# sanje2v/DualSuperResLearningForSemSeg

Measured on AMD Instinct MI355X. Metric: stage-3 train images/sec at 256x512->512x1024, higher is better.
Workload: dtype f32; 1 GPU; DSRL stage 3 (ResNet-101 OS16 + ASPP + SSSR/SISR decoders + FA loss), full train step, random-init weights, 256x512 input -> 512x1024 logits; global_batch=8, per_gpu_batch=8, parallelism=dp1, optimizer=SGD m0.9 wd5e-4 lr0.006

## Files before the change

dualsuperreslearningforsemseg_amd/csrc/conv_igemm.hip:

```cpp
#include "common.h"
#include "conv_common.h"
#include <algorithm>
#include <atomic>
#include <stdlib.h>
#include <string.h>
#include <mutex>
#include <vector>

namespace dsrl {

static std::atomic<int> g_conv_precision{-1};
constexpr int BK = 32;
constexpr int LDS_LD = 36;

template <int MR, int NR, int WGM, int WGN, bool DGRAD, int MINW = 2, bool = false>
__global__ __launch_bounds__(256, MINW) void conv_igemm_f32_kernel(const ConvArgs a) {
    constexpr int BM = 32 * MR * WGM, BN = 32 * NR * WGN;
    constexpr int A_IT = BM / 32, B_IT = BN / 32;
    extern __shared__ __attribute__((aligned(16))) float smem[];

    const int tid = threadIdx.x;
    const int lane = tid & 63;
    const int wave = __builtin_amdgcn_readfirstlane(tid >> 6);
    const int wm = wave / WGN, wn = wave % WGN;
// ... 1468 lines not shown
struct DgradBn { const float* x; const float* y; const float* mean; const float* invstd; float* stats; int ldx, ldy, relu; float gscale = 1.f; };
static bool bn_y_ok(const float* y, int ldy, int relu, int N, int H, int W, int C) {
    if (relu == 2) return y != nullptr && C % 32 == 0 && (long long)ldy >= (long long)N * H * W && ((uintptr_t)y % 4) == 0;
    return relu == 0 || (relu == 1 && y != nullptr && ldy >= C);
}
static int dgrad_impl(const float* dy, int lddy, const float* w, const float* wt_in, float* dx, int lddx,
                      int N, int H, int W, int C, int K, int R, int S, int stride, int pad, int dil,
                      void* ws, size_t ws_bytes, dsrl_stream_t stream, int accumulate, const DgradBn* bn = nullptr,
                      const unsigned* dy_amax = nullptr, const unsigned* w_amax = nullptr, const void* wt_split = nullptr,
                      const void* dy_planes = nullptr, const void* wt_planes = nullptr) {
    if (int e = check_conv(dy, w, dx, N, H, W, C, K, R, S, stride, pad, dil)) return e;
    const int Kp = pad4(K);
    DSRL_REQUIRE(lddy % 4 == 0 && ((uintptr_t)dy % 16) == 0, DSRL_E_UNSUPPORTED,
                 "conv2d_dgrad: lddy (%d) must be a multiple of 4 and dy 16-byte aligned", lddy);
    DSRL_REQUIRE(lddy >= Kp && lddx >= C, DSRL_E_BADARG, "conv2d_dgrad: ld smaller than (padded) channel count");
    hipStream_t st = (hipStream_t)stream;
    if (int e = bind_stream_device(st)) return e;
    const int Ho = out_size(H, R, stride, pad, dil), Wo = out_size(W, S, stride, pad, dil);
    const FwdPlan p = plan_dgrad(N, Ho, Wo, Kp, C, R, S, H, W, conv_planes(PASS_DGRAD), stride);
    const size_t wtb = dgrad_wt_bytes(C, K, R, S);
    DSRL_REQUIRE(ws && ws_bytes >= wtb + p.ws, DSRL_E_WORKSPACE, "conv2d_dgrad: workspace %zu < %zu", ws_bytes, wtb + p.ws);
    const float* wt = wt_in;
    float* slabs = (float*)((char*)ws + wtb);
    const bool use_planes = conv_f16() && dy_planes != nullptr && wt_planes != nullptr && dy_amax != nullptr && w_amax != nullptr && stride == 1 && K % 8 == 0 &&
                            planes_usable(K, lddy, dy_planes, wt_planes) && planes_cfg_supported((int)p.cfg, p.kg) && !(p.coop && p.splits > 1);
    const bool use_split = conv_f16() && wt_split != nullptr && w_amax != nullptr;
    if (wt == nullptr && use_planes) wt = (const float*)wt_planes;
    if (wt == nullptr && use_split) wt = (const float*)wt_split;
    if (wt == nullptr) {
        hipLaunchKernelGGL(weight_transpose_kernel, dim3((unsigned)ceil_div(C, 32), (unsigned)ceil_div(Kp, 32), (unsigned)(R * S)), dim3(256), 0, st,
                           w, (float*)ws, K, Kp, R * S, C);
        if (int e = launch_status("weight_transpose_kernel")) return e;
        wt = (const float*)ws;
    }
    ConvArgs a{};
    a.x = dy; a.w = wt; a.ldx = lddy; a.N = N; a.H = Ho; a.W = Wo; a.C = Kp; a.K = C; a.R = R; a.S = S; a.Ho = H; a.Wo = W;
    a.stride = stride; a.pad = pad; a.dil = dil; a.M = p.M; a.cchunks = p.cchunks; a.splits = p.splits; a.kg = p.kg; a.slab = (long long)p.M * C;
    {
        const long long xb = span_bytes((long long)N * Ho * Wo, lddy, Kp), wb = (long long)C * R * S * Kp * 4, yb = p.splits > 1 ? (long long)p.M * C * 4 : span_bytes(p.M, lddx, C);
        DSRL_REQUIRE_31(xb, "conv2d_dgrad(dy)"); DSRL_REQUIRE_31(wb, "conv2d_dgrad(w)"); DSRL_REQUIRE_31(yb, "conv2d_dgrad(dx)");
        a.x_bytes = (unsigned)xb; a.w_bytes = (unsigned)wb; a.y_bytes = (unsigned)yb;
    }
    if (conv_f16()) {
        OperandAmax am{dy_amax, w_amax};
        if (int e = resolve_amax(am, dy, lddy, (long long)N * Ho * Wo, Kp, w, C, (long long)K * R * S, C, ws, ws_bytes, wtb + p.ws, st, "conv2d_dgrad")) return e;
        a.amax_a = am.a; a.amax_b = am.b;
        if (wt_split != nullptr && w_amax != nullptr) {
            DSRL_REQUIRE(((uintptr_t)wt_split % 16) == 0, DSRL_E_BADARG, "conv2d_dgrad: unaligned pre-split filter");
            a.w = (const float*)wt_split; a.w_split = 1;
        }
        if (use_planes) {
            const long long pe = (long long)N * Ho * Wo * lddy, we = (long long)C * R * S * K;
            a.planes = conv_planes(PASS_DGRAD); a.w_split = 0;
            a.x = (const float*)dy_planes; a.w = (const float*)wt_planes;
            a.x_bytes = (unsigned)(span_bytes((long long)N * Ho * Wo, lddy, K) / 2); a.w_bytes = (unsigned)(we * 2);
            a.a_lo = (unsigned)planes_lo_offset(pe); a.b_lo = (unsigned)planes_lo_offset(we);
        }
    }
    ProfScope prof(prof_family(PASS_DGRAD), 2.0 * (double)dsrl_conv2d_inbounds_macs(N, H, W, C, K, R, S, stride, pad, dil), 4.0 * ((double)N * H * W * C + (double)K * R * S * C + (double)N * out_size(H, R, stride, pad, dil) * out_size(W, S, stride, pad, dil) * K), st);
    prof.shape("dgrad", N, H, W, C, K, R, stride, pad, dil);
    if (p.splits > 1 && !(p.coop && a.amax_a != nullptr && !a.planes && stride == 1)) {
        DSRL_REQUIRE(bn == nullptr, DSRL_E_UNSUPPORTED, "conv2d_dgrad: BatchNorm sums asked from a split-K launch that reduces through slabs");
        a.y = slabs; a.ldy = C; a.bias = nullptr;
        if (int e = launch_igemm<true>(a, p.cfg, st)) return e;
        const long long total = (long long)p.M * C;
        hipLaunchKernelGGL(splitk_reduce_kernel, dim3((unsigned)std::min<long long>(ceil_div(total, 256), 4096)), dim3(256), 0, st,
                           (const float*)slabs, p.splits, a.slab, p.M, C, (const float*)nullptr, dx, lddx, accumulate);
        return launch_status("splitk_reduce_kernel");
    }
    if (p.splits > 1) {
        a.coop_slab = slabs; a.tickets = const_cast<unsigned*>(a.amax_a);
        a.y_bytes = (unsigned)span_bytes(p.M, lddx, C);
    }
    a.y = dx; a.ldy = lddx; a.bias = nullptr; a.accumulate = accumulate;
    if (stride > 1 && conv_planes(PASS_DGRAD) && H % stride == 0 && W % stride == 0 && (W / stride) % 32 == 0 && knob("DSRL_DGRAD_PARITY", 1)) {
        int bm, bn_; cfg_dims(p.cfg, bm, bn_);
        const long long Mc = (long long)N * (H / stride) * (W / stride);
        if (Mc % bm == 0) { a.par = stride; a.Hh = H / stride; a.Wh = W / stride; a.pbm = bm; }
    }
    if (bn) {
        a.bn_x = bn->x; a.bn_y = bn->y; a.bn_mean = bn->mean; a.bn_invstd = bn->invstd; a.bstats = bn->stats; a.bn_ldx = bn->ldx; a.bn_ldy = bn->ldy; a.bn_relu = bn->relu;
        a.bn_gscale = bn->gscale;
        const bool y4 = bn->relu != 1 || (bn->ldy % 4 == 0 && ((uintptr_t)bn->y % 16) == 0);
        a.bn_fast = a.par == 0 && C % 4 == 0 && bn->ldx % 4 == 0 && y4 && ((uintptr_t)bn->x % 16) == 0 &&
                    ((uintptr_t)bn->mean % 16) == 0 && ((uintptr_t)bn->invstd % 16) == 0 && ((uintptr_t)bn->stats % 16) == 0;
    }
    return launch_igemm<true>(a, p.cfg, st);
}

extern "C" int dsrl_conv2d_dgrad(const float* dy, int lddy, const float* w, const float* wt_in, float* dx, int lddx,
                                 int N, int H, int W, int C, int K, int R, int S, int stride, int pad, int dil,
                                 void* ws, size_t ws_bytes, dsrl_stream_t stream) {
    return dgrad_impl(dy, lddy, w, wt_in, dx, lddx, N, H, W, C, K, R, S, stride, pad, dil, ws, ws_bytes, stream, 0);
}
extern "C" int dsrl_conv2d_dgrad_stats_parts(int N, int H, int W, int C, int K, int R, int S, int stride, int pad, int dil) {
    const int Ho = out_size(H, R, stride, pad, dil), Wo = out_size(W, S, stride, pad, dil);
    if (Ho <= 0 || Wo <= 0) return 0;
    const int npl = conv_planes(PASS_DGRAD);
    return fwd_stats_parts(plan_dgrad(N, Ho, Wo, pad4(K), C, R, S, H, W, npl, stride), npl, true);
}
extern "C" int dsrl_conv2d_dgrad_bnstats(const float* dy, int lddy, const float* w, const float* wt_in, float* dx, int lddx,
                                         int N, int H, int W, int C, int K, int R, int S, int stride, int pad, int dil,
                                         void* ws, size_t ws_bytes, const float* bn_x, int bn_ldx, const float* bn_y, int bn_ldy,
                                         const float* bn_mean, const float* bn_invstd, int bn_relu, float* bstats, int stats_parts, int accumulate,
                                         dsrl_stream_t stream) {
    DSRL_REQUIRE(bn_x && bn_mean && bn_invstd && bstats && bn_ldx >= C && bn_y_ok(bn_y, bn_ldy, bn_relu, N, H, W, C), DSRL_E_BADARG, "conv2d_dgrad_bnstats: bad BatchNorm arguments");
    DSRL_REQUIRE(dsrl_conv2d_dgrad_stats_parts(N, H, W, C, K, R, S, stride, pad, dil) == stats_parts && stats_parts > 0, DSRL_E_BADARG,
                 "conv2d_dgrad_bnstats: this launch writes %d row blocks of partials, the caller expects %d",
                 dsrl_conv2d_dgrad_stats_parts(N, H, W, C, K, R, S, stride, pad, dil), stats_parts);
    DgradBn bn{bn_x, bn_y, bn_mean, bn_invstd, bstats, bn_ldx, bn_ldy, bn_relu};
    return dgrad_impl(dy, lddy, w, wt_in, dx, lddx, N, H, W, C, K, R, S, stride, pad, dil, ws, ws_bytes, stream, accumulate ? 1 : 0, &bn);
}
extern "C" int dsrl_conv2d_dgrad_accumulate(const float* dy, int lddy, const float* w, const float* wt_in, float* dx, int lddx,
                                            int N, int H, int W, int C, int K, int R, int S, int stride, int pad, int dil,
                                            void* ws, size_t ws_bytes, dsrl_stream_t stream) {
    return dgrad_impl(dy, lddy, w, wt_in, dx, lddx, N, H, W, C, K, R, S, stride, pad, dil, ws, ws_bytes, stream, 1);
}

static void launch_wgrad(const WgradArgs& a_in, TileCfg cfg, int bm, int bn, dim3 grid, hipStream_t st) {
    const int npl = conv_planes(PASS_WGRAD);
    const bool f16 = conv_f16();
    if (npl) {
        WgradArgs a = a_in;
        make_magic(a.Ho * a.Wo, a.mHW, a.sHW);
        make_magic(a.Wo, a.mW, a.sW);
        const size_t stages = (size_t)2 * npl * 16 * ((bm * 2 + 64) + (bn * 2 + 64));
        const int kg = a.kg > 1 ? a.kg : 1;
        if (kg > 1) {
            const size_t lds = std::max(stages * kg, (size_t)kg * (bm / 32) * (bn / 32) / 4 * 16384 + 8192);
#define DSRL_LAUNCH_WKG(a_, b_, c_, d_, NPL_, KG_, F16_)                                                                            \
            {                                                                                                                        \
                static const hipError_t attr = hipFuncSetAttribute((const void*)conv_wgrad_split_kernel<a_, b_, c_, d_, NPL_, KG_, F16_>,  \
                                                                   hipFuncAttributeMaxDynamicSharedMemorySize, 144 * 1024);          \
                (void)attr;                                                                                                          \
                hipLaunchKernelGGL((conv_wgrad_split_kernel<a_, b_, c_, d_, NPL_, KG_, F16_>), grid, dim3(256 * KG_), lds, st, a);   \
            }
#define DSRL_WKG_BY_NPL(a_, b_, c_, d_, KG_) { if (f16 && npl == 1) DSRL_LAUNCH_WKG(a_, b_, c_, d_, 1, KG_, true) else if (f16) DSRL_LAUNCH_WKG(a_, b_, c_, d_, 2, KG_, true) else if (npl == 2) DSRL_LAUNCH_WKG(a_, b_, c_, d_, 2, KG_, false) else DSRL_LAUNCH_WKG(a_, b_, c_, d_, 3, KG_, false) }
            if (cfg == T64x64) DSRL_WKG_BY_NPL(1, 1, 2, 2, 2)
            else if (cfg == T128x64) DSRL_WKG_BY_NPL(2, 1, 2, 2, 2)
            else if (cfg == T64x128) DSRL_WKG_BY_NPL(1, 2, 2, 2, 2)
            else DSRL_WKG_BY_NPL(2, 2, 2, 2, 2)
#undef DSRL_WKG_BY_NPL
#undef DSRL_LAUNCH_WKG
            return;
        }
        const size_t lds = stages;
#define DSRL_LAUNCH_WGRAD(a_, b_, c_, d_)                                                                           \
        if (f16 && npl == 1) hipLaunchKernelGGL((conv_wgrad_split_kernel<a_, b_, c_, d_, 1, 1, true>), grid, dim3(256), lds, st, a); \
        else if (f16) hipLaunchKernelGGL((conv_wgrad_split_kernel<a_, b_, c_, d_, 2, 1, true>), grid, dim3(256), lds, st, a); \
        else if (npl == 2) hipLaunchKernelGGL((conv_wgrad_split_kernel<a_, b_, c_, d_, 2>), grid, dim3(256), lds, st, a); \
        else hipLaunchKernelGGL((conv_wgrad_split_kernel<a_, b_, c_, d_, 3>), grid, dim3(256), lds, st, a);
        DSRL_CFG_SWITCH(cfg, DSRL_LAUNCH_WGRAD)
#undef DSRL_LAUNCH_WGRAD
        return;
    }
    const size_t lds = (size_t)32 * (bm + bn) * sizeof(float);
#define DSRL_LAUNCH_WGRAD(a_, b_, c_, d_) hipLaunchKernelGGL((conv_wgrad_f32_kernel<a_, b_, c_, d_>), grid, dim3(256), lds, st, a_in)
    DSRL_CFG_SWITCH(cfg, DSRL_LAUNCH_WGRAD)
#undef DSRL_LAUNCH_WGRAD
}

namespace dsrl {
struct WgPlan { int Ho, Wo; long long P; TileCfg cfg; int bm, bn, ktiles, ctiles, psplits; TapList tl; size_t ws; bool w3; };
static int w3_psplits(long long tiles, long long chunks) {
    const int forced = knob("DSRL_FORCE_PSPLITS", 0);
    if (forced > 0) return (int)std::max<long long>(1, std::min<long long>(forced, chunks));
    long long sp = std::max<long long>(1, 2 * kNumCU / std::max<long long>(tiles, 1));
// ... 518 lines not shown
```

dualsuperreslearningforsemseg_amd/csrc/conv_split_kernel.h:

```cpp
#pragma once
#include "common.h"
#include "conv_common.h"

namespace dsrl {

template <int MR, int NR, int WGM, int WGN, bool DGRAD, int NPL, int KG = 1, int ARITH = 0, bool STR1 = false, bool COOP = false>
__global__ __launch_bounds__(64 * WGM * WGN * KG, KG == 1 ? 2 : 1)
void conv_igemm_split_kernel(const ConvArgs a) {
    const int stride = STR1 ? 1 : a.stride, par = STR1 ? 0 : a.par;
    constexpr bool F16 = ARITH != 0, PREB = ARITH == 2;
    constexpr int NT = 64 * WGM * WGN, RP = NT / 4;
    static_assert(NT == 256 || (NT == 512 && KG == 1), "4 waves per K group, or one group of 8 waves");
    static_assert(!F16 || NPL <= 2, "f16x3 carries two fp16 terms per operand, f16x1 one");
    using PT = Plane<F16>;
    using pl4 = typename PT::v4; using pl8 = typename PT::v8;
    const unsigned am_a = F16 ? amax_fetch(a.amax_a) : 0u, am_b = F16 ? amax_fetch(a.amax_b) : 0u;
    int sh_a = 0, sh_b = 0;
    constexpr int BM = 32 * MR * WGM, BN = 32 * NR * WGN;
    constexpr int A_IT = (BM + RP - 1) / RP, B_IT = (BN + RP - 1) / RP;
    constexpr int NV = A_IT + B_IT;
    constexpr bool FS = F16;
    constexpr int ROWB = FS ? 64 : 32;
    constexpr int STAGE = (BM + BN) * NPL * ROWB;
    extern __shared__ __attribute__((aligned(16))) float smem[];
    const int grp = KG > 1 ? __builtin_amdgcn_readfirstlane((int)(threadIdx.x >> 8)) : 0;
    char* const S0 = reinterpret_cast<char*>(smem) + grp * 2 * STAGE;
    char* const S1 = S0 + STAGE;

    const int tid = threadIdx.x & (NT - 1);
    const int lane = tid & 63;
    const int wave = __builtin_amdgcn_readfirstlane(tid >> 6);
    const int wm = wave / WGN, wn = wave % WGN;
    const int tile = a.xcd_remap ? xcd_contiguous(blockIdx.x, a.mtiles * a.ntiles) : blockIdx.x;
    const int tile_m = fast_div(tile, a.mNT, a.sNT);
    const int m0 = tile_m * BM, n0 = (tile - tile_m * a.ntiles) * BN, z = blockIdx.z;
    const int HoWo = a.Ho * a.Wo;

    const int c4 = tid & 3, r0 = tid >> 2;
    const bool b_rows = (BN % RP == 0) || r0 < BN;
    int a_n[A_IT], a_h[A_IT], a_w[A_IT];
    bool a_ok[A_IT];
#pragma unroll
    for (int i = 0; i < A_IT; ++i) {
        const int m = m0 + r0 + RP * i;
        a_ok[i] = m < a.M && (BM % RP == 0 || r0 + RP * i < BM);
        const int mm = a_ok[i] ? ((DGRAD && par) ? dgrad_pix(a, m) : m) : 0;
        const int n = fast_div(mm, a.mHW, a.sHW), rem = mm - n * HoWo;
        const int ho = fast_div(rem, a.mW, a.sW), wo = rem - ho * a.Wo;
        a_n[i] = n;
        if (DGRAD) { a_h[i] = ho + a.pad; a_w[i] = wo + a.pad; }
        else { a_h[i] = ho * stride - a.pad; a_w[i] = wo * stride - a.pad; }
    }
    const int RS = a.R * a.S;
    const __amdgpu_buffer_rsrc_t xr = __builtin_amdgcn_make_buffer_rsrc((void*)a.x, 0, (int)a.x_bytes, 0x00020000);
    const __amdgpu_buffer_rsrc_t wr = __builtin_amdgcn_make_buffer_rsrc((void*)a.w, 0, (int)a.w_bytes, 0x00020000);
    unsigned b_off[B_IT];
#pragma unroll
    for (int i = 0; i < B_IT; ++i) {
        const int k = n0 + r0 + RP * i;
        b_off[i] = (k < a.K && b_rows) ? (unsigned)k * (unsigned)(RS * a.C) * 4u : kOOB;
    }

    unsigned long long tapmask = 0ull;
    if (a.R * a.S == 1 && a.pad == 0) {
        tapmask = 1ull;
    } else {
        const int mf = m0, ml = min(m0 + BM, a.M) - 1;
        const int nf = fast_div(mf, a.mHW, a.sHW), nl = fast_div(ml, a.mHW, a.sHW);
        int hf = 0, hl = a.Ho - 1, wf = 0, wl = a.Wo - 1;
        if (nf == nl) {
            hf = fast_div(mf - nf * HoWo, a.mW, a.sW); hl = fast_div(ml - nl * HoWo, a.mW, a.sW);
            if (hf == hl) { wf = (mf - nf * HoWo) - hf * a.Wo; wl = (ml - nl * HoWo) - hl * a.Wo; }
        }
        const int pcls = (DGRAD && par) ? (m0 / BM) % (par * par) : 0;
        const int ph = (DGRAD && par) ? pcls / par : 0, pw = (DGRAD && par) ? pcls - ph * par : 0;
        if (DGRAD && par) { hf = 0; hl = a.Ho - 1; wf = 0; wl = a.Wo - 1; }
        for (int r = 0; r < a.R; ++r)
            for (int s = 0; s < a.S; ++s) {
                bool act;
                if (DGRAD) {
                    act = (hl + a.pad - r * a.dil >= 0) && (hf + a.pad - r * a.dil <= (a.H - 1) * stride) &&
                          (wl + a.pad - s * a.dil >= 0) && (wf + a.pad - s * a.dil <= (a.W - 1) * stride);
                    if (par) act = act && ((ph + a.pad - r * a.dil) % par == 0) && ((pw + a.pad - s * a.dil) % par == 0);
                } else {
                    act = (hl * stride - a.pad + r * a.dil >= 0) && (hf * stride - a.pad + r * a.dil <= a.H - 1) &&
                          (wl * stride - a.pad + s * a.dil >= 0) && (wf * stride - a.pad + s * a.dil <= a.W - 1);
                }
                if (act) tapmask |= 1ull << (r * a.S + s);
            }
    }
    const int ntaps = __builtin_popcountll(tapmask);
    const int nq = ntaps * a.cchunks;
    int q0 = 0, q1 = nq;
    if (a.splits > 1) { q0 = (int)((long long)nq * z / a.splits); q1 = (int)((long long)nq * (z + 1) / a.splits); }

    f32x16 acc[MR][NR];
#pragma unroll
    for (int i = 0; i < MR; ++i)
#pragma unroll
        for (int j = 0; j < NR; ++j)
#pragma unroll
            for (int e = 0; e < 16; ++e) acc[i][j][e] = 0.f;

    int cc = 0, tap = 0, pos = q0;
    unsigned long long rem_mask = tapmask;
    if (q0 < q1) {
        if (q0 > 0) {
            int skip = q0 / a.cchunks;
            cc = q0 - skip * a.cchunks;
            while (skip--) rem_mask &= rem_mask - 1;
        }
        tap = __builtin_ctzll(rem_mask);
    }
    auto advance = [&](int n) {
        cc += n; pos += n;
        while (cc >= a.cchunks) { cc -= a.cchunks; rem_mask &= rem_mask - 1; tap = __builtin_ctzll(rem_mask); }
    };
    unsigned a_off[A_IT];
    const unsigned inv_s = 65536u / (unsigned)a.S + 1u;
    auto set_tap = [&](int t) {
        const int r = a.S <= 8 ? (int)(((unsigned)t * inv_s) >> 16) : t / a.S, s = t - r * a.S;
#pragma unroll
        for (int i = 0; i < A_IT; ++i) {
            int hi, wi; bool ok = a_ok[i];
            if (DGRAD) {
                const int hn = a_h[i] - r * a.dil, wn_ = a_w[i] - s * a.dil;
                hi = hn / stride; wi = wn_ / stride;
                ok = ok && hn >= 0 && wn_ >= 0 && hi * stride == hn && wi * stride == wn_ && hi < a.H && wi < a.W;
            } else {
                hi = a_h[i] + r * a.dil; wi = a_w[i] + s * a.dil;
                ok = ok && hi >= 0 && hi < a.H && wi >= 0 && wi < a.W;
            }
            a_off[i] = ok ? (unsigned)((a_n[i] * a.H + hi) * a.W + wi) * (unsigned)a.ldx * 4u : kOOB;
        }
    };
    float4 R0[NV][2], R1[NV][2];
#pragma unroll
    for (int v = 0; v < NV; ++v) { R0[v][0] = R0[v][1] = R1[v][0] = R1[v][1] = make_float4(0.f, 0.f, 0.f, 0.f); }
    auto gload = [&](float4 (*R)[2], int t, int ch, unsigned dead) {
#pragma unroll
        for (int hf = 0; hf < 2; ++hf) {
            const int c = ch * 32 + hf * 16 + c4 * 4;
            const unsigned coff = (c < a.C ? (unsigned)c * 4u : kOOB) | dead;
            const unsigned woff = __builtin_elementwise_add_sat(coff, (unsigned)(t * a.C) * 4u);
#pragma unroll
            for (int i = 0; i < A_IT; ++i) R[i][hf] = buf_load4(xr, __builtin_elementwise_add_sat(a_off[i], coff));
#pragma unroll
            for (int i = 0; i < B_IT; ++i) R[A_IT + i][hf] = buf_load4(wr, __builtin_elementwise_add_sat(b_off[i], woff));
        }
    };
    int nextq = q0 + grp, tap_set = -1;
    auto issue = [&](float4 (*R)[2]) {
        const bool live = nextq < q1;
        if (live) {
            advance(nextq - pos);
            if (tap != tap_set) { set_tap(tap); tap_set = tap; }
            nextq += KG;
        }
        gload(R, tap, cc, live ? 0u : kOOB);
    };

    const int frag_row = lane & 31;
    auto wswz = [&](int hf) -> int { return FS ? (((((hf << 1) | (c4 >> 1)) ^ ((r0 >> 2) & 3)) << 4) + ((c4 & 1) << 3)) : ((((c4 >> 1) ^ ((r0 >> 3) & 1)) << 4) + ((c4 & 1) << 3)); };
    auto rswz = [&](int hf) -> int { return FS ? ((((hf << 1) | (lane >> 5)) ^ ((frag_row >> 2) & 3)) << 4) : (((lane >> 5) ^ ((frag_row >> 3) & 1)) << 4); };
    float res[4] = {0.f, 0.f, 0.f, 0.f};
    auto cstep = [&](char* nb, float4 (*R)[2], int hf, int c) {
        const int v = c / NPL, pl = c % NPL;
        if (PREB && v >= A_IT) {
            if (pl == 0 && b_rows) {
                const float4 x = R[v][hf];
                char* q = nb + (NPL * BM + r0 + RP * (v - A_IT)) * ROWB + wswz(hf);
                *reinterpret_cast<uint2*>(q) = make_uint2(__float_as_uint(x.x), __float_as_uint(x.y));
                if (NPL > 1) *reinterpret_cast<uint2*>(q + BN * ROWB) = make_uint2(__float_as_uint(x.z), __float_as_uint(x.w));
// ... 207 lines not shown
            const unsigned toff = (unsigned)threadIdx.x * 16u;
            constexpr int kSC1 = 16;
#pragma unroll
            for (int v = 0; v < NV4; ++v) {
                u32x4 q;
#pragma unroll
                for (int e = 0; e < 4; ++e) {
                    const int f = 4 * v + e;
                    q[e] = __float_as_uint(share(f / (NSH / (MR * NR)) / NR, f / (NSH / (MR * NR)) % NR, f % (NSH / (MR * NR))));
                }
                __builtin_amdgcn_raw_buffer_store_b128(q, sr, (int)(toff + (unsigned)v * (unsigned)(NTH * 16) + (unsigned)z * zstride), 0, kSC1);
            }
            asm volatile("s_waitcnt vmcnt(0)" ::: "memory");
            __shared__ int coop_last;
            __syncthreads();
            if (threadIdx.x == 0) {
                unsigned* tk = a.tickets + coop_ticket_word(tile);
                const unsigned old = __hip_atomic_fetch_add(tk, 1u, __ATOMIC_RELAXED, __HIP_MEMORY_SCOPE_AGENT);
                const int last = old == (unsigned)(a.splits - 1);
                if (last) __hip_atomic_store(tk, 0u, __ATOMIC_RELAXED, __HIP_MEMORY_SCOPE_AGENT);
                coop_last = last;
            }
            __syncthreads();
            if (!coop_last) return;
            float tot[NSH];
#pragma unroll
            for (int f = 0; f < NSH; ++f) tot[f] = 0.f;
            constexpr int ZB = NV4 > 8 ? 1 : 4;
            for (int z0 = 0; z0 < a.splits; z0 += ZB) {
                u32x4 in[ZB][NV4];
#pragma unroll
                for (int d = 0; d < ZB; ++d) {
                    const int zz = z0 + d;
                    const unsigned zoff = (zz < a.splits && zz != z) ? (unsigned)zz * zstride : kOOB;
#pragma unroll
                    for (int v = 0; v < NV4; ++v)
                        in[d][v] = __builtin_amdgcn_raw_buffer_load_b128(sr, (int)__builtin_elementwise_add_sat(zoff, toff + (unsigned)v * (unsigned)(NTH * 16)), 0, kSC1);
                }
#pragma unroll
                for (int d = 0; d < ZB; ++d) {
                    const int zz = z0 + d;
                    if (zz < a.splits) {
#pragma unroll
                        for (int f = 0; f < NSH; ++f) {
                            const float own = share(f / (NSH / (MR * NR)) / NR, f / (NSH / (MR * NR)) % NR, f % (NSH / (MR * NR)));
                            const float v = zz == z ? own : __uint_as_float(in[d][f / 4][f % 4]);
                            tot[f] = zz == 0 ? v : tot[f] + v;
                        }
                    }
                }
            }
#pragma unroll
            for (int f = 0; f < NSH; ++f) {
                const int i = f / (NSH / (MR * NR)) / NR, j = f / (NSH / (MR * NR)) % NR, e = f % (NSH / (MR * NR));
                if constexpr (KG > 1) mine[i][j][e] = tot[f]; else acc[i][j][e] = tot[f];
            }
            if constexpr (KG > 1) {
                if (!DGRAD && a.stats != nullptr) {
                    float* xch = reinterpret_cast<float*>(smem);
                    __syncthreads();
#pragma unroll
                    for (int i = 0; i < MR; ++i)
#pragma unroll
                        for (int j = 0; j < NR; ++j)
#pragma unroll
                            for (int k = 0; k < EPG; ++k) xch[((i * NR + j) * 16 + grp * EPG + k) * 256 + tid] = mine[i][j][k];
                    __syncthreads();
                    if (grp == 0) {
#pragma unroll
                        for (int i = 0; i < MR; ++i)
#pragma unroll
                            for (int j = 0; j < NR; ++j)
#pragma unroll
                                for (int e = 0; e < 16; ++e) acc[i][j][e] = xch[((i * NR + j) * 16 + e) * 256 + tid];
                    }
                }
            }
        }
    }
    const bool single = coop || a.splits == 1;
    float* yout = a.y + (!single ? (long long)z * a.slab : 0ll);
    const __amdgpu_buffer_rsrc_t yr = __builtin_amdgcn_make_buffer_rsrc((void*)yout, 0, (int)a.y_bytes, 0x00020000);
    const int col = lane & 31, rq = (lane >> 5) * 4 + rowg;
#pragma unroll
    for (int j = 0; j < NR; ++j) {
        const int k = n0 + (wn * NR + j) * 32 + col;
        const bool kok = k < a.K;
        const float bv = (a.bias != nullptr && kok) ? a.bias[k] : 0.f;
#pragma unroll
        for (int i = 0; i < MR; ++i) {
            const int mb32 = m0 + (wm * MR + i) * 32, mb = mb32 + rq;
            const int pix0 = (DGRAD && par) ? dgrad_pix(a, min(mb32, a.M - 1)) : mb32, pst = (DGRAD && par) ? par : 1;
            if (a.accumulate && single) {
                float old[EPG];
#pragma unroll
                for (int e = 0; e < EPG; ++e) {
                    const int m = mb + (e & 3) + 8 * (e >> 2);
                    const unsigned off = (kok && m < a.M) ? ((unsigned)(pix0 + (m - mb32) * pst) * (unsigned)a.ldy + (unsigned)k) * 4u : kOOB;
                    old[e] = __uint_as_float(__builtin_amdgcn_raw_buffer_load_b32(yr, (int)off, 0, 0));
                }
#pragma unroll
                for (int e = 0; e < EPG; ++e) share_add(i, j, e, old[e]);
            }
#pragma unroll
            for (int e = 0; e < EPG; ++e) {
                const int m = mb + (e & 3) + 8 * (e >> 2);
                const unsigned off = (kok && m < a.M) ? ((unsigned)(pix0 + (m - mb32) * pst) * (unsigned)a.ldy + (unsigned)k) * 4u : kOOB;
                __builtin_amdgcn_raw_buffer_store_b32(__float_as_uint(share(i, j, e) + bv), yr, (int)off, 0, 0);
            }
        }
    }
    bool bstats_done = false;
    if constexpr (DGRAD && KG == 1) {
        if (a.bstats != nullptr && single && a.bn_fast) {
            constexpr int TR = 32 * MR, TC = 32 * NR, CQ = TC / 4, RSTEP = 64 / CQ, NIT = TR / RSTEP, NB = NIT < 8 ? NIT : 8;
            float* wt = reinterpret_cast<float*>(smem) + (size_t)wave * TR * TC;
            __syncthreads();
#pragma unroll
            for (int i = 0; i < MR; ++i)
#pragma unroll
                for (int j = 0; j < NR; ++j)
#pragma unroll
                    for (int e = 0; e < 16; ++e)
                        wt[(i * 32 + (e & 3) + 8 * (e >> 2) + 4 * (lane >> 5)) * TC + j * 32 + (lane & 31)] = acc[i][j][e];
            const int c4 = lane % CQ, r0_ = lane / CQ;
            const int kk = n0 + wn * TC + 4 * c4;
            const bool kok4 = kk < a.K;
            const float4 mu4 = kok4 ? *reinterpret_cast<const float4*>(a.bn_mean + kk) : make_float4(0.f, 0.f, 0.f, 0.f);
            const float4 is4 = kok4 ? *reinterpret_cast<const float4*>(a.bn_invstd + kk) : make_float4(0.f, 0.f, 0.f, 0.f);
            float sg[4] = {0.f, 0.f, 0.f, 0.f}, sgx[4] = {0.f, 0.f, 0.f, 0.f};
            const int mrow0 = m0 + wm * TR;
#pragma unroll
            for (int b0 = 0; b0 < NIT; b0 += NB) {
                float4 xv[NB], yv[NB];
#pragma unroll
                for (int u = 0; u < NB; ++u) {
                    const int m = mrow0 + r0_ + RSTEP * (b0 + u);
                    const bool ok = kok4 && m < a.M;
                    xv[u] = ok ? *reinterpret_cast<const float4*>(a.bn_x + (long long)m * a.bn_ldx + kk) : make_float4(0.f, 0.f, 0.f, 0.f);
                    if (a.bn_relu == 2) yv[u] = bn_mask4(ok ? bn_mask_word(a, kk, m) >> (kk & 31) : 15u);
                    else yv[u] = (ok && a.bn_relu) ? *reinterpret_cast<const float4*>(a.bn_y + (long long)m * a.bn_ldy + kk) : make_float4(1.f, 1.f, 1.f, 1.f);
                }
#pragma unroll
                for (int u = 0; u < NB; ++u) {
                    const int row = r0_ + RSTEP * (b0 + u);
                    if (kok4 && mrow0 + row < a.M) {
                        const float4 gv = *reinterpret_cast<const float4*>(wt + row * TC + 4 * c4);
                        const float gs = a.bn_gscale;
                        const float g0 = (a.bn_relu && !(yv[u].x > 0.f)) ? 0.f : gv.x * gs, g1 = (a.bn_relu && !(yv[u].y > 0.f)) ? 0.f : gv.y * gs;
                        const float g2 = (a.bn_relu && !(yv[u].z > 0.f)) ? 0.f : gv.z * gs, g3 = (a.bn_relu && !(yv[u].w > 0.f)) ? 0.f : gv.w * gs;
                        sg[0] += g0; sgx[0] += g0 * ((xv[u].x - mu4.x) * is4.x);
                        sg[1] += g1; sgx[1] += g1 * ((xv[u].y - mu4.y) * is4.y);
                        sg[2] += g2; sgx[2] += g2 * ((xv[u].z - mu4.z) * is4.z);
                        sg[3] += g3; sgx[3] += g3 * ((xv[u].w - mu4.w) * is4.w);
                    }
                }
            }
#pragma unroll
            for (int sft = CQ; sft < 64; sft <<= 1)
#pragma unroll
                for (int q = 0; q < 4; ++q) { sg[q] += __shfl_xor(sg[q], sft); sgx[q] += __shfl_xor(sgx[q], sft); }
            if (lane < CQ && kok4) {
                const int nparts = a.mtiles * WGM, part = tile_m * WGM + wm;
                float* o = a.bstats + (long long)part * a.K + kk;
                *reinterpret_cast<float4*>(o) = make_float4(sg[0], sg[1], sg[2], sg[3]);
                *reinterpret_cast<float4*>(o + (long long)nparts * a.K) = make_float4(sgx[0], sgx[1], sgx[2], sgx[3]);
            }
            bstats_done = true;
        }
    }
    if (DGRAD && a.bstats != nullptr && single && !bstats_done) {
        const int nparts = a.mtiles * WGM, part = tile_m * WGM + wm;
        float* ex = reinterpret_cast<float*>(smem) + (size_t)KG * MR * NR * 4 * 256 * 4;
#pragma unroll
        for (int j = 0; j < NR; ++j) {
            const int k = n0 + (wn * NR + j) * 32 + col;
            const bool kok = k < a.K;
            const float mu = kok ? a.bn_mean[k] : 0.f, is = kok ? a.bn_invstd[k] : 0.f;
            float sg = 0.f, sgx = 0.f;
#pragma unroll
            for (int i = 0; i < MR; ++i) {
                float xv[EPG], yv[EPG];
                const int mb32 = m0 + (wm * MR + i) * 32;
                const int pix0 = par ? dgrad_pix(a, min(mb32, a.M - 1)) : mb32, pst = par ? par : 1;
#pragma unroll
                for (int e = 0; e < EPG; ++e) {
                    const int m = mb32 + rq + (e & 3) + 8 * (e >> 2);
                    const bool ok = kok && m < a.M;
                    const long long px = pix0 + (m - mb32) * pst;
                    xv[e] = ok ? a.bn_x[px * a.bn_ldx + k] : 0.f;
                    if (a.bn_relu == 2) yv[e] = (!ok || ((bn_mask_word(a, k, px) >> (k & 31)) & 1u)) ? 1.f : 0.f;
                    else yv[e] = (ok && a.bn_relu) ? a.bn_y[px * a.bn_ldy + k] : 1.f;
                }
#pragma unroll
                for (int e = 0; e < EPG; ++e) {
                    const int m = mb32 + rq + (e & 3) + 8 * (e >> 2);
                    if (kok && m < a.M) {
                        const float g = (a.bn_relu && !(yv[e] > 0.f)) ? 0.f : share(i, j, e) * a.bn_gscale;
                        sg += g; sgx += g * ((xv[e] - mu) * is);
                    }
                }
            }
            sg += __shfl_xor(sg, 32); sgx += __shfl_xor(sgx, 32);
            if (KG == 1) {
                if (lane < 32 && kok) {
                    float* o = a.bstats + (long long)part * a.K + k;
                    o[0] = sg; o[(long long)nparts * a.K] = sgx;
                }
            } else if (lane < 32) {
                ex[(((grp * 4 + wave) * NR + j) * 2 + 0) * 32 + lane] = sg;
                ex[(((grp * 4 + wave) * NR + j) * 2 + 1) * 32 + lane] = sgx;
            }
        }
        if constexpr (KG > 1) {
            __syncthreads();
            if (grp == 0 && lane < 32) {
#pragma unroll
                for (int j = 0; j < NR; ++j) {
                    const int k = n0 + (wn * NR + j) * 32 + col;
                    float sg = 0.f, sgx = 0.f;
#pragma unroll
                    for (int g = 0; g < KG; ++g) {
                        sg += ex[(((g * 4 + wave) * NR + j) * 2 + 0) * 32 + lane];
                        sgx += ex[(((g * 4 + wave) * NR + j) * 2 + 1) * 32 + lane];
                    }
                    if (k < a.K) {
                        float* o = a.bstats + (long long)part * a.K + k;
                        o[0] = sg; o[(long long)nparts * a.K] = sgx;
                    }
                }
            }
        }
    }
    const bool stats_wave = !(KG > 1 && grp > 0);
    if (a.stats != nullptr && single) {
        const int nparts = a.mtiles, part = tile_m;
        float* mg = reinterpret_cast<float*>(smem) + (KG > 1 ? (size_t)KG * MR * NR * 4 * 256 * 4 : 0);
        float sn[NR], sm[NR], sq[NR];
        if (stats_wave) {
#pragma unroll
// ... 54 lines not shown
```

Baseline: 509.6 images/s.

## Skip dead parity-class dgrad tiles and allow fused BN stats under parity decomposition

Parity-class dgrad tiles of strided convs whose tap set is empty now take a shortcut. They exit early when accumulating without BN stats. With BN stats they skip the LDS transpose and the read-modify-write of the output, reading the existing output rows directly to compute the BN backward partial sums. It also removes the restriction that disabled the fast fused-BN-stats path when parity decomposition is active, using parity-aware pixel indexing. This avoids wasted epilogue stores and loads for 1x1 stride-2 dgrad tiles, at the cost of extra branching and code size.

Result: no change. 512.9 images/s (median of 6 runs) (+0.6%).

```diff
diff --git a/dualsuperreslearningforsemseg_amd/csrc/conv_igemm.hip b/dualsuperreslearningforsemseg_amd/csrc/conv_igemm.hip
--- a/dualsuperreslearningforsemseg_amd/csrc/conv_igemm.hip
+++ b/dualsuperreslearningforsemseg_amd/csrc/conv_igemm.hip
@@ -1574,7 +1574,7 @@
         a.bn_x = bn->x; a.bn_y = bn->y; a.bn_mean = bn->mean; a.bn_invstd = bn->invstd; a.bstats = bn->stats; a.bn_ldx = bn->ldx; a.bn_ldy = bn->ldy; a.bn_relu = bn->relu;
         a.bn_gscale = bn->gscale;
         const bool y4 = bn->relu != 1 || (bn->ldy % 4 == 0 && ((uintptr_t)bn->y % 16) == 0);
-        a.bn_fast = a.par == 0 && C % 4 == 0 && bn->ldx % 4 == 0 && y4 && ((uintptr_t)bn->x % 16) == 0 &&
+        a.bn_fast = C % 4 == 0 && bn->ldx % 4 == 0 && y4 && ((uintptr_t)bn->x % 16) == 0 &&
                     ((uintptr_t)bn->mean % 16) == 0 && ((uintptr_t)bn->invstd % 16) == 0 && ((uintptr_t)bn->stats % 16) == 0;
     }
     return launch_igemm<true>(a, p.cfg, st);
diff --git a/dualsuperreslearningforsemseg_amd/csrc/conv_split_kernel.h b/dualsuperreslearningforsemseg_amd/csrc/conv_split_kernel.h
--- a/dualsuperreslearningforsemseg_amd/csrc/conv_split_kernel.h
+++ b/dualsuperreslearningforsemseg_amd/csrc/conv_split_kernel.h
@@ -1,4 +1,5 @@
 #pragma once
+#include <type_traits>
 #include "common.h"
 #include "conv_common.h"
 
@@ -62,8 +63,9 @@
     }
 
     unsigned long long tapmask = 0ull;
+    const int pcls = (DGRAD && par) ? tile_m % (par * par) : 0;
     if (a.R * a.S == 1 && a.pad == 0) {
-        tapmask = 1ull;
+        tapmask = pcls == 0 ? 1ull : 0ull;
     } else {
         const int mf = m0, ml = min(m0 + BM, a.M) - 1;
         const int nf = fast_div(mf, a.mHW, a.sHW), nl = fast_div(ml, a.mHW, a.sHW);
@@ -72,7 +74,6 @@
             hf = fast_div(mf - nf * HoWo, a.mW, a.sW); hl = fast_div(ml - nl * HoWo, a.mW, a.sW);
             if (hf == hl) { wf = (mf - nf * HoWo) - hf * a.Wo; wl = (ml - nl * HoWo) - hl * a.Wo; }
         }
-        const int pcls = (DGRAD && par) ? (m0 / BM) % (par * par) : 0;
         const int ph = (DGRAD && par) ? pcls / par : 0, pw = (DGRAD && par) ? pcls - ph * par : 0;
         if (DGRAD && par) { hf = 0; hl = a.Ho - 1; wf = 0; wl = a.Wo - 1; }
         for (int r = 0; r < a.R; ++r)
@@ -89,6 +90,8 @@
                 if (act) tapmask |= 1ull << (r * a.S + s);
             }
     }
+    const bool dead = DGRAD && !STR1 && tapmask == 0ull && a.splits == 1;
+    if (dead && a.accumulate && a.bstats == nullptr) return;
     const int ntaps = __builtin_popcountll(tapmask);
     const int nq = ntaps * a.cchunks;
     int q0 = 0, q1 = nq;
@@ -462,6 +465,8 @@
     float* yout = a.y + (!single ? (long long)z * a.slab : 0ll);
     const __amdgpu_buffer_rsrc_t yr = __builtin_amdgcn_make_buffer_rsrc((void*)yout, 0, (int)a.y_bytes, 0x00020000);
     const int col = lane & 31, rq = (lane >> 5) * 4 + rowg;
+    const bool dead_fast = dead && KG == 1 && a.bstats != nullptr && a.bn_fast && (a.ldy & 3) == 0 && (reinterpret_cast<uintptr_t>(a.y) & 15) == 0;
+    const bool keep_old = dead && a.accumulate;
 #pragma unroll
     for (int j = 0; j < NR; ++j) {
         const int k = n0 + (wn * NR + j) * 32 + col;
@@ -471,7 +476,7 @@
         for (int i = 0; i < MR; ++i) {
             const int mb32 = m0 + (wm * MR + i) * 32, mb = mb32 + rq;
             const int pix0 = (DGRAD && par) ? dgrad_pix(a, min(mb32, a.M - 1)) : mb32, pst = (DGRAD && par) ? par : 1;
-            if (a.accumulate && single) {
+            if (a.accumulate && single && !dead_fast) {
                 float old[EPG];
 #pragma unroll
                 for (int e = 0; e < EPG; ++e) {
@@ -482,6 +487,7 @@
 #pragma unroll
                 for (int e = 0; e < EPG; ++e) share_add(i, j, e, old[e]);
             }
+            if (keep_old) continue;
 #pragma unroll
             for (int e = 0; e < EPG; ++e) {
                 const int m = mb + (e & 3) + 8 * (e >> 2);
@@ -494,15 +500,26 @@
     if constexpr (DGRAD && KG == 1) {
         if (a.bstats != nullptr && single && a.bn_fast) {
             constexpr int TR = 32 * MR, TC = 32 * NR, CQ = TC / 4, RSTEP = 64 / CQ, NIT = TR / RSTEP, NB = NIT < 8 ? NIT : 8;
+            static_assert(32 % RSTEP == 0, "a lane's rows of one pass lie in one 32-row block");
             float* wt = reinterpret_cast<float*>(smem) + (size_t)wave * TR * TC;
-            __syncthreads();
-#pragma unroll
-            for (int i = 0; i < MR; ++i)
-#pragma unroll
-                for (int j = 0; j < NR; ++j)
-#pragma unroll
-                    for (int e = 0; e < 16; ++e)
-                        wt[(i * 32 + (e & 3) + 8 * (e >> 2) + 4 * (lane >> 5)) * TC + j * 32 + (lane & 31)] = acc[i][j][e];
+            if (!dead_fast) {
+                __syncthreads();
+#pragma unroll
+                for (int i = 0; i < MR; ++i)
+#pragma unroll
+                    for (int j = 0; j < NR; ++j)
+#pragma unroll
+                        for (int e = 0; e < 16; ++e)
+                            wt[(i * 32 + (e & 3) + 8 * (e >> 2) + 4 * (lane >> 5)) * TC + j * 32 + (lane & 31)] = acc[i][j][e];
+            }
+            int pixb[MR];
+#pragma unroll
+            for (int i = 0; i < MR; ++i) {
+                const int mb32 = m0 + (wm * MR + i) * 32;
+                pixb[i] = par ? dgrad_pix(a, min(mb32, a.M - 1)) : mb32;
+            }
+            const int pst = par ? par : 1;
+            const bool old_rows = dead_fast && a.accumulate;
             const int c4 = lane % CQ, r0_ = lane / CQ;
             const int kk = n0 + wn * TC + 4 * c4;
             const bool kok4 = kk < a.K;
@@ -510,32 +527,40 @@
             const float4 is4 = kok4 ? *reinterpret_cast<const float4*>(a.bn_invstd + kk) : make_float4(0.f, 0.f, 0.f, 0.f);
             float sg[4] = {0.f, 0.f, 0.f, 0.f}, sgx[4] = {0.f, 0.f, 0.f, 0.f};
             const int mrow0 = m0 + wm * TR;
-#pragma unroll
-            for (int b0 = 0; b0 < NIT; b0 += NB) {
-                float4 xv[NB], yv[NB];
-#pragma unroll
-                for (int u = 0; u < NB; ++u) {
-                    const int m = mrow0 + r0_ + RSTEP * (b0 + u);
-                    const bool ok = kok4 && m < a.M;
-                    xv[u] = ok ? *reinterpret_cast<const float4*>(a.bn_x + (long long)m * a.bn_ldx + kk) : make_float4(0.f, 0.f, 0.f, 0.f);
-                    if (a.bn_relu == 2) yv[u] = bn_mask4(ok ? bn_mask_word(a, kk, m) >> (kk & 31) : 15u);
-                    else yv[u] = (ok && a.bn_relu) ? *reinterpret_cast<const float4*>(a.bn_y + (long long)m * a.bn_ldy + kk) : make_float4(1.f, 1.f, 1.f, 1.f);
-                }
-#pragma unroll
-                for (int u = 0; u < NB; ++u) {
-                    const int row = r0_ + RSTEP * (b0 + u);
-                    if (kok4 && mrow0 + row < a.M) {
-                        const float4 gv = *reinterpret_cast<const float4*>(wt + row * TC + 4 * c4);
-                        const float gs = a.bn_gscale;
-                        const float g0 = (a.bn_relu && !(yv[u].x > 0.f)) ? 0.f : gv.x * gs, g1 = (a.bn_relu && !(yv[u].y > 0.f)) ? 0.f : gv.y * gs;
-                        const float g2 = (a.bn_relu && !(yv[u].z > 0.f)) ? 0.f : gv.z * gs, g3 = (a.bn_relu && !(yv[u].w > 0.f)) ? 0.f : gv.w * gs;
-                        sg[0] += g0; sgx[0] += g0 * ((xv[u].x - mu4.x) * is4.x);
-                        sg[1] += g1; sgx[1] += g1 * ((xv[u].y - mu4.y) * is4.y);
-                        sg[2] += g2; sgx[2] += g2 * ((xv[u].z - mu4.z) * is4.z);
-                        sg[3] += g3; sgx[3] += g3 * ((xv[u].w - mu4.w) * is4.w);
-                    }
-                }
-            }
+            auto bn_rows = [&](auto old_tag) {
+                constexpr bool OLD = decltype(old_tag)::value;
+                constexpr int NBv = OLD ? (NB < 4 ? NB : 4) : NB;
+#pragma unroll
+                for (int b0 = 0; b0 < NIT; b0 += NBv) {
+                    float4 xv[NBv], yv[NBv], ov[OLD ? NBv : 1];
+#pragma unroll
+                    for (int u = 0; u < NBv; ++u) {
+                        const int ib = RSTEP * (b0 + u) / 32, row = r0_ + RSTEP * (b0 + u);
+                        const bool ok = kok4 && mrow0 + row < a.M;
+                        const long long px = pixb[ib] + (row - 32 * ib) * pst;
+                        xv[u] = ok ? *reinterpret_cast<const float4*>(a.bn_x + px * a.bn_ldx + kk) : make_float4(0.f, 0.f, 0.f, 0.f);
+                        if (a.bn_relu == 2) yv[u] = bn_mask4(ok ? bn_mask_word(a, kk, px) >> (kk & 31) : 15u);
+                        else yv[u] = (ok && a.bn_relu) ? *reinterpret_cast<const float4*>(a.bn_y + px * a.bn_ldy + kk) : make_float4(1.f, 1.f, 1.f, 1.f);
+                        if constexpr (OLD) ov[u] = (ok && old_rows) ? *reinterpret_cast<const float4*>(a.y + px * a.ldy + kk) : make_float4(0.f, 0.f, 0.f, 0.f);
+                    }
+#pragma unroll
+                    for (int u = 0; u < NBv; ++u) {
+                        const int row = r0_ + RSTEP * (b0 + u);
+                        if (kok4 && mrow0 + row < a.M) {
+                            float4 gv;
+                            if constexpr (OLD) gv = ov[u]; else gv = *reinterpret_cast<const float4*>(wt + row * TC + 4 * c4);
+                            const float gs = a.bn_gscale;
+                            const float g0 = (a.bn_relu && !(yv[u].x > 0.f)) ? 0.f : gv.x * gs, g1 = (a.bn_relu && !(yv[u].y > 0.f)) ? 0.f : gv.y * gs;
+                            const float g2 = (a.bn_relu && !(yv[u].z > 0.f)) ? 0.f : gv.z * gs, g3 = (a.bn_relu && !(yv[u].w > 0.f)) ? 0.f : gv.w * gs;
+                            sg[0] += g0; sgx[0] += g0 * ((xv[u].x - mu4.x) * is4.x);
+                            sg[1] += g1; sgx[1] += g1 * ((xv[u].y - mu4.y) * is4.y);
+                            sg[2] += g2; sgx[2] += g2 * ((xv[u].z - mu4.z) * is4.z);
+                            sg[3] += g3; sgx[3] += g3 * ((xv[u].w - mu4.w) * is4.w);
+                        }
+                    }
+                }
+            };
+            if (dead_fast) bn_rows(std::true_type{}); else bn_rows(std::false_type{});
 #pragma unroll
             for (int sft = CQ; sft < 64; sft <<= 1)
 #pragma unroll
```
